# pierrepaleo/sift_pyocl

Measured on AMD Instinct MI355X. Metric: SiftPlan.keypoints throughput, 4096x4096 fp32 (Mpix/s; keypoints/s in keypoints_per_s), higher is better.
Workload: dtype f32

## Files before the change

include/siftmi.h:

```cpp
#ifndef SIFTMI_H
#define SIFTMI_H

#include <stdint.h>

#ifdef __cplusplus
extern "C" {
#endif

#define SIFTMI_OK 0
#define SIFTMI_EINVAL (-1)
#define SIFTMI_ENOMEM (-2)
#define SIFTMI_EDEVICE (-3)
#define SIFTMI_ECAPACITY (-4)

enum siftmi_dtype {
    SIFTMI_F32 = 0, SIFTMI_U8 = 1, SIFTMI_U16 = 2, SIFTMI_U32 = 3, SIFTMI_U64 = 4,
    SIFTMI_I32 = 5, SIFTMI_I64 = 6, SIFTMI_F64 = 7, SIFTMI_RGB8 = 8
};

typedef struct siftmi_keypoint {
    float x, y, scale, angle;
    uint8_t desc[128];
} siftmi_keypoint;

// ... 203 lines not shown
int siftmi_stage_dog(int32_t device_id, const float *blur_a, const float *blur_b, float *out, int64_t n);
int siftmi_stage_local_maxmin(int32_t device_id, const float *blurs, int32_t W, int32_t H, int32_t octsize,
                              const siftmi_params *params, float *out, int64_t capacity, int64_t *n_out);
int siftmi_stage_interp(int32_t device_id, const float *blurs, int32_t W, int32_t H, const float *cand, int64_t n,
                        const siftmi_params *params, float *out, int32_t *out_scale, int64_t *n_out);
#define SIFTMI_STAGE_GUARD 64
int siftmi_stage_detect_ex(int32_t device_id, const float *blurs, int32_t W, int32_t H, int32_t octsize,
                           const siftmi_params *params, int32_t form, int32_t rows, int32_t xcd_map, int32_t y_lo, int32_t y_hi,
                           int64_t cand_capacity, int64_t kp_capacity, float *cand, float *kp, int32_t *kp_aux,
                           int32_t *counters);
#define SIFTMI_STAGE_TOP_FILL 0x7fc5a5a5u
int siftmi_stage_detect_lazy(int32_t device_id, const float *blurs5, const float *top_taps, int32_t n_taps, int32_t W, int32_t H,
                             int32_t octsize, const siftmi_params *params, int32_t rows, int32_t xcd_map, int32_t y_lo, int32_t y_hi,
                             int64_t cand_capacity, int64_t kp_capacity, float *cand, float *kp, int32_t *kp_aux,
                             int32_t *counters, float *plane5);
int siftmi_stage_compact(int32_t device_id, const float *kps, int64_t n, int64_t start, int64_t end, float *out, int64_t *n_out);
int siftmi_stage_gradient(int32_t device_id, const float *img, float *grad, float *ori, int32_t W, int32_t H);
int siftmi_stage_orientation(int32_t device_id, const float *blurs, int32_t W, int32_t H, int32_t octsize,
                             const float *kps, const int32_t *kp_scale, int64_t n, const siftmi_params *params,
                             float *out, int32_t *out_scale, int64_t capacity, int64_t *n_out);
int siftmi_stage_descriptor(int32_t device_id, const float *blurs, int32_t W, int32_t H, int32_t octsize,
                            const float *kps, const int32_t *kp_scale, int64_t n, uint8_t *desc);
int siftmi_stage_orientation_ex(int32_t device_id, const float *blurs, int32_t W, int32_t H, int32_t octsize,
                                const float *kps, const int32_t *kp_scale, int64_t n, const siftmi_params *params,
                                float *out, int32_t *out_scale, int64_t capacity, int64_t *n_out,
                                int32_t form, int32_t blocks, int32_t *form_used);
int siftmi_stage_descriptor_ex(int32_t device_id, const float *blurs, int32_t W, int32_t H, int32_t octsize,
                               const float *kps, const int32_t *kp_scale, int64_t n, uint8_t *desc,
                               int32_t form, int32_t blocks, int32_t *form_used);
int siftmi_stage_gradient_maps(int32_t device_id, const float *planes, int32_t n_oct, const int32_t *W, const int32_t *H,
// ... 11 lines not shown
```

sift_pyocl_amd/_lib.py:

```python
import ctypes as C
import os
import subprocess

HERE = os.path.dirname(os.path.abspath(__file__))
LIB_PATH = os.path.join(HERE, "libsiftmi.so")

OK, EINVAL, ENOMEM, EDEVICE, ECAPACITY = 0, -1, -2, -3, -4
METRIC_L1, METRIC_L2SQ = 0, 1
INTERP_MODE, INTERP_CUBIC = 0, 1
INTERPS = {None: INTERP_MODE, "linear": INTERP_MODE, "cubic": INTERP_CUBIC}


def interp_code(interp, mode=1, rgb=False):
    if not (interp is None or isinstance(interp, str)) or interp not in INTERPS:
        raise ValueError("interp must be None, 'linear' or 'cubic', not %r" % (interp,))
    code = INTERPS[interp]
    if code == INTERP_CUBIC and int(mode) != 1:
        raise ValueError("interp='cubic' takes mode=1 only (other values are reserved), not %r" % (mode,))
    if code == INTERP_CUBIC and rgb:
        raise ValueError("interp='cubic' takes float32 frames; an RGB plan has no cubic sampler")
    return code


def interp_keyword(impl):
# ... 151 lines not shown
    "siftmi_stage_blur_ex": (C.c_int, [C.c_int32, C.c_void_p, C.c_int32, C.c_void_p, C.c_int32, C.c_int32, C.c_void_p, C.c_int32,
                                       C.c_int32, C.c_int32, C.c_int32, C.POINTER(C.c_int32)]),
    "siftmi_stage_blur_handoff": (C.c_int, [C.c_int32, C.c_void_p, C.c_void_p, C.c_void_p, C.c_int32, C.c_int32, C.c_void_p, C.c_int32,
                                            C.c_int32, C.c_int32, C.POINTER(C.c_int32)]),
    "siftmi_stage_dog": (C.c_int, [C.c_int32, C.c_void_p, C.c_void_p, C.c_void_p, C.c_int64]),
    "siftmi_stage_local_maxmin": (C.c_int, [C.c_int32, C.c_void_p, C.c_int32, C.c_int32, C.c_int32, C.POINTER(Params),
                                            C.c_void_p, C.c_int64, C.POINTER(C.c_int64)]),
    "siftmi_stage_interp": (C.c_int, [C.c_int32, C.c_void_p, C.c_int32, C.c_int32, C.c_void_p, C.c_int64,
                                      C.POINTER(Params), C.c_void_p, C.c_void_p, C.POINTER(C.c_int64)]),
    "siftmi_stage_detect_ex": (C.c_int, [C.c_int32, C.c_void_p, C.c_int32, C.c_int32, C.c_int32, C.POINTER(Params), C.c_int32,
                                         C.c_int32, C.c_int32, C.c_int32, C.c_int32, C.c_int64, C.c_int64, C.c_void_p, C.c_void_p,
                                         C.c_void_p, C.c_void_p]),
    "siftmi_stage_detect_lazy": (C.c_int, [C.c_int32, C.c_void_p, C.c_void_p, C.c_int32, C.c_int32, C.c_int32, C.c_int32, C.POINTER(Params),
                                           C.c_int32, C.c_int32, C.c_int32, C.c_int32, C.c_int64, C.c_int64, C.c_void_p, C.c_void_p,
                                           C.c_void_p, C.c_void_p, C.c_void_p]),
    "siftmi_stage_compact": (C.c_int, [C.c_int32, C.c_void_p, C.c_int64, C.c_int64, C.c_int64, C.c_void_p, C.POINTER(C.c_int64)]),
    "siftmi_stage_gradient": (C.c_int, [C.c_int32, C.c_void_p, C.c_void_p, C.c_void_p, C.c_int32, C.c_int32]),
    "siftmi_stage_orientation": (C.c_int, [C.c_int32, C.c_void_p, C.c_int32, C.c_int32, C.c_int32, C.c_void_p,
                                           C.c_void_p, C.c_int64, C.POINTER(Params), C.c_void_p, C.c_void_p,
                                           C.c_int64, C.POINTER(C.c_int64)]),
    "siftmi_stage_descriptor": (C.c_int, [C.c_int32, C.c_void_p, C.c_int32, C.c_int32, C.c_int32, C.c_void_p,
                                          C.c_void_p, C.c_int64, C.c_void_p]),
    "siftmi_stage_orientation_ex": (C.c_int, [C.c_int32, C.c_void_p, C.c_int32, C.c_int32, C.c_int32, C.c_void_p,
                                              C.c_void_p, C.c_int64, C.POINTER(Params), C.c_void_p, C.c_void_p,
                                              C.c_int64, C.POINTER(C.c_int64), C.c_int32, C.c_int32, C.POINTER(C.c_int32)]),
    "siftmi_stage_descriptor_ex": (C.c_int, [C.c_int32, C.c_void_p, C.c_int32, C.c_int32, C.c_int32, C.c_void_p,
                                             C.c_void_p, C.c_int64, C.c_void_p, C.c_int32, C.c_int32, C.POINTER(C.c_int32)]),
    "siftmi_stage_gradient_maps": (C.c_int, [C.c_int32, C.c_void_p, C.c_int32, C.c_void_p, C.c_void_p, C.c_int32,
                                             C.c_int32, C.c_int32, C.c_void_p, C.c_void_p]),
    "siftmi_plan_records_device": (C.c_int, [C.c_void_p, C.POINTER(C.c_void_p), C.POINTER(C.c_int64)]),
# ... 96 lines not shown
```

sift_pyocl_amd/csrc/k_extrema.hpp:

```cpp
#pragma once
#include <hip/hip_runtime.h>
#include <stdint.h>
#include "siftmath.hpp"
#include "k_xcd.hpp"
#include <type_traits>

namespace siftk {

struct BlurPlanes { const float *p[6]; };

#define SIFT_EXT_ROWS 64
inline int extrema_strip_rows(int W, int H, int border, int min_strips = 2000) {
    const int nx = (W - 2 * border + 61) / 62;
    int rows = SIFT_EXT_ROWS;
    while (rows > 4 && (int64_t)nx * ((H - 2 * border + rows - 1) / rows) < min_strips) rows >>= 1;
    return rows;
}

__device__ __forceinline__ float dog_at(const BlurPlanes &b, int s, size_t pos) { return b.p[s][pos] - b.p[s + 1][pos]; }

#ifndef SIFT_EXT_WAVES
#define SIFT_EXT_WAVES 5
#endif
#define SIFT_EXT_BUF 128
template <int BUF> struct ExtWaveLdsT { float4 buf[BUF + 192]; };
using ExtWaveLds = ExtWaveLdsT<SIFT_EXT_BUF>;

struct RefineArgs {
    float peak_thresh, init_sigma;
    float4 *kp;
    int *kp_aux, *n_kp;
    int kp_capacity, oct;
    int *c_scale;
};
__device__ __forceinline__ void refine_candidates(const BlurPlanes &b, int W, int H, const float4 *__restrict__ cand, int n,
                                                  float peak_thresh, float init_sigma, float4 *__restrict__ kp,
                                                  int *__restrict__ kp_aux, int *__restrict__ n_kp, int kp_capacity, int oct,
                                                  int first, int stride, int *__restrict__ c_scale);

template <int BUF>
__device__ __forceinline__ void ext_store_pending(const ExtWaveLdsT<BUF> &L, float4 *__restrict__ cand, int capacity, int slot, int count, int lane) {
    __builtin_amdgcn_wave_barrier();
    for (int e = lane; e < count; e += 64)
        if (slot + e < capacity) cand[slot + e] = L.buf[e];
    __builtin_amdgcn_wave_barrier();
}

template <int BUF>
__device__ __forceinline__ void ext_edge_filter(const BlurPlanes &b, int W, float edth, ExtWaveLdsT<BUF> &L, int from, int &pending, int lane) {
    int out = from;
    __builtin_amdgcn_wave_barrier();
    for (int base = from; base < pending; base += 64) {
        const int e = base + lane;
        bool keep = false;
        float4 c = make_float4(0.f, 0.f, 0.f, 0.f);
        if (e < pending) {
            c = L.buf[e];
            const float val = c.x;
            const int s = (int)c.w;
// ... 106 lines not shown
        for (int k = 0; k < 3; k++) {
            const unsigned long long m = __ballot(found[k]);
            if (m) {
                if (found[k]) L.buf[pending + __popcll(m & ((1ull << lane) - 1ull))] = make_float4(ctr[k], (float)yc, (float)x, (float)(k + 1));
                pending += __popcll(m);
            }
        }
        if (pending > BUF) {
            ext_edge_filter(b, W, edth, L, tested, pending, lane);
            tested = 0;
            if (REFINE) refine_parked();
            else {
                int slot = 0;
                if (lane == 0) slot = atomicAdd(counter, pending);
                ext_store_pending(L, cand, capacity, __shfl(slot, 0), pending, lane);
                pending = 0;
            }
        }
#pragma unroll
        for (int k = 0; k < 3; k++) ctr[k] = ctr_next[k];
    }
    ext_edge_filter(b, W, edth, L, tested, pending, lane);
    if (REFINE) refine_parked();
}

template <bool REFINE, bool LAZY = false>
__global__ __launch_bounds__(256) __attribute__((amdgpu_waves_per_eu(REFINE ? 4 : SIFT_EXT_WAVES, 8))) void extrema_kernel(BlurPlanes b, int W, int H, int border, int rows, double contrast,
                                                      float edth, float4 *__restrict__ cand,
                                                      int *__restrict__ counter, int capacity, RefineArgs ra,
                                                      int y_lo, int y_hi,
// ... 12 lines not shown
    extrema_strip<SIFT_EXT_BUF, REFINE, LAZY>(b, W, H, border, rows, active, active ? wid % nx : 0, active ? wid / nx : 0, contrast, edth, cand,
                                        counter, capacity, L, pending, &ra, y_lo, y_hi);
    if (REFINE) return;
    if (lane == 0) s_pending[threadIdx.x >> 6] = pending;
    __syncthreads();
    if (threadIdx.x == 0) {
        const int tot = s_pending[0] + s_pending[1] + s_pending[2] + s_pending[3];
        s_base = tot ? atomicAdd(counter, tot) : 0;
    }
    __syncthreads();
    {
        const int w = threadIdx.x >> 6;
        int slot = s_base;
        for (int q = 0; q < w; q++) slot += s_pending[q];
        ext_store_pending(L, cand, capacity, slot, pending, lane);
    }
}

__device__ __forceinline__ void refine_candidates(const BlurPlanes &b, int W, int H, const float4 *__restrict__ cand, int n,
                                                  float peak_thresh, float init_sigma, float4 *__restrict__ kp,
                                                  int *__restrict__ kp_aux, int *__restrict__ n_kp, int kp_capacity, int oct,
                                                  int first, int stride, int *__restrict__ c_scale) {
    int seen[3] = {0, 0, 0};
    for (int i = first; i < n; i += stride) {
        const float4 k = cand[i];
        int r = (int)k.y, c = (int)k.z;
        const int scale = (int)k.w;
        if (r == -1) continue;
        seen[0] += scale <= 1; seen[1] += scale == 2; seen[2] += scale >= 3;
        const float *Pa = b.p[0], *Pb = b.p[1], *Pc = b.p[2], *Pd = b.p[3];
// ... 101 lines not shown
```

sift_pyocl_amd/csrc/k_keypoint.hpp:

```cpp
#pragma once
#include <hip/hip_runtime.h>
#include <stdint.h>
#include "k_extrema.hpp"
#include "siftmath.hpp"

namespace siftk {

struct KpRecord { float x, y, scale, angle; uint8_t desc[128]; };
static_assert(sizeof(KpRecord) == 144, "record layout");

struct GradTaps { float xa, xb, ya, yb; bool bx, by; };

__device__ __forceinline__ GradTaps gradient_fetch(const float *__restrict__ I, int x, int y, int W, int H) {
    const size_t pos = (size_t)y * W + x;
    GradTaps t;
    t.bx = (x == 0) || (x == W - 1);
    t.by = (y == 0) || (y == H - 1);
    t.xa = I[x == W - 1 ? pos : pos + 1];
    t.xb = I[x == 0 ? pos : pos - 1];
    t.ya = I[y == 0 ? pos : pos - W];
    t.yb = I[y == H - 1 ? pos : pos + W];
    return t;
}

// ... 18 lines not shown
    return q;
}

#define SIFT_MAX_OCTAVES 24
#define SIFT_GROUPS 3
struct Counters {
    int n_rec;
    int tail_timeout;
    unsigned rec_word[SIFT_GROUPS];
    int g_kp[SIFT_GROUPS];
    int g_out[SIFT_GROUPS];
    int desc_next[SIFT_GROUPS];
    int n_cand[SIFT_MAX_OCTAVES + 1];
    int c_scale[SIFT_MAX_OCTAVES][3];
    int o_scale[SIFT_MAX_OCTAVES][3];
    uint32_t mm[2];
    int tail_ready[8];
};

struct OctaveTable {
    const float *base;
    long long off[SIFT_MAX_OCTAVES];
    int W[SIFT_MAX_OCTAVES], H[SIFT_MAX_OCTAVES];
    const float *gmap, *omap;
};
__device__ __forceinline__ size_t map_offset(const OctaveTable &tab, int oct, int scale) {
    return (size_t)(tab.off[oct] / 2) + (size_t)(scale - 1) * tab.W[oct] * tab.H[oct];
}

struct alignas(16) RecordSink {
// ... 621 lines not shown
```

sift_pyocl_amd/csrc/k_top_patch.hpp:

```cpp
#pragma once
#include <hip/hip_runtime.h>
#include <stdint.h>
#include "k_pyramid.hpp"

namespace siftk {

#define SIFT_TOP_R 6
#define SIFT_TOP_P (2 * SIFT_TOP_R + 1)
struct TopTaps { float t[64]; };

inline size_t top_patch_lds_bytes(int n_taps) {
    const size_t win = (size_t)(SIFT_TOP_P - 1 + n_taps);
    return (win * win + win * SIFT_TOP_P + 64 + SIFT_TOP_P * SIFT_TOP_P) * sizeof(float);
}

__global__ __launch_bounds__(64) void top_patch_kernel(const float *__restrict__ p4, float *__restrict__ p5, int W, int H, TopTaps taps, int n_taps,
                                                       float4 *__restrict__ cand, const int *__restrict__ n_cand, int cand_capacity) {
    extern __shared__ float top_lds[];
    const int lane = threadIdx.x;
    const int C = (n_taps & 1) ? n_taps / 2 : n_taps / 2 - 1;
    const int WIN = SIFT_TOP_P - 1 + n_taps;
    float *win = top_lds;
    float *hb = win + WIN * WIN;
    float *tr = hb + WIN * SIFT_TOP_P;
    float *pt = tr + 64;
    if (lane < n_taps) tr[lane] = taps.t[n_taps - 1 - lane];
    const int n = min(*n_cand, cand_capacity);
    for (int i = blockIdx.x; i < n; i += gridDim.x) {
        const float4 k = cand[i];
        const int r = __builtin_amdgcn_readfirstlane((int)k.y), c = __builtin_amdgcn_readfirstlane((int)k.z);
        if (__builtin_amdgcn_readfirstlane((int)k.w) != 3 || r == -1) continue;
        __syncthreads();
        const int y0 = r - SIFT_TOP_R, x0 = c - SIFT_TOP_R;
        for (int wc = lane; wc < WIN; wc += 64) {
            const float *col = p4 + reflect_index(x0 - C + wc, W);
#pragma unroll 8
            for (int wr = 0; wr < WIN; wr++) win[wr * WIN + wc] = col[(size_t)reflect_index(y0 - C + wr, H) * W];
        }
        __syncthreads();
        for (int base = 0; base < WIN * SIFT_TOP_P; base += 64 * 4) {
            const float *src[4];
            float a[4];
#pragma unroll
            for (int j = 0; j < 4; j++) {
                const int idx = min(base + 64 * j + lane, WIN * SIFT_TOP_P - 1);
                const int wr = idx / SIFT_TOP_P;
                src[j] = win + wr * WIN + (idx - wr * SIFT_TOP_P);
                a[j] = 0.0f;
            }
            for (int q = 0; q < n_taps; q++) {
                const float t = tr[q];
#pragma unroll
// ... 42 lines not shown
```

sift_pyocl_amd/csrc/siftmi.hip:

```cpp
#include <hip/hip_runtime.h>
#include <hip/hip_ext.h>

#include <cmath>
#include <cstdlib>
#include <cstring>
#include <algorithm>
#include <chrono>
#include <mutex>
#include <new>
#include <string>
#include <vector>

#include "host_common.hpp"
#include "k_extrema.hpp"
#include "k_keypoint.hpp"
#include "k_descriptor.hpp"
#include "k_align.hpp"
#include "k_align_batch.hpp"
#include "k_warp_cubic.hpp"
#include "k_stack.hpp"
#include "k_stack_clip.hpp"
#include "k_stack_accum.hpp"
#include "k_pyramid.hpp"
#include "k_tail.hpp"
// ... 88 lines not shown
size_t dtype_size(int dt) {
    switch (dt) {
        case SIFTMI_F32: return 4; case SIFTMI_U8: return 1; case SIFTMI_U16: return 2; case SIFTMI_U32: return 4;
        case SIFTMI_U64: return 8; case SIFTMI_I32: return 4; case SIFTMI_I64: return 8; case SIFTMI_F64: return 8;
        case SIFTMI_RGB8: return 3;
    }
    return 0;
}

}

struct GroupLists {
    float4 *kp = nullptr;  int *kp_aux = nullptr;  int64_t cap_kp = 0;
    float4 *okp = nullptr; int *oaux = nullptr;    int64_t cap_out = 0;
    float4 *cand = nullptr; int64_t cap_cand = 0;
};

struct siftmi_plan {
    void *chain = nullptr;
    int device = 0;
    hipStream_t stream = nullptr;
    int H = 0, W = 0, dtype = 0;
    siftmi_params par{};
    Options opt;
    int profile = 0;
    int n_oct = 0;
    std::vector<int> ow, oh;
    int64_t kpsize = 0;
    int64_t bytes = 0;
    float *planes = nullptr;
// ... 49 lines not shown
    KpRecord *host_out = nullptr;
    int host_cap = 0;
    bool desc_rows = true;
    Taps taps[6];
    bool have_init = false;
    std::vector<Event> events;
    size_t n_events = 0;
    hipEvent_t ev_first = nullptr, ev_last[3] = {nullptr, nullptr, nullptr};
    float last_min = 0, last_max = 0;
    int64_t last_count = 0;
    int last_overflow = 0;
    bool last_valid = false;
    int last_tail_first = 0;
    int last_n_cand[SIFT_MAX_OCTAVES] = {0};
    int last_c_scale[SIFT_MAX_OCTAVES][3] = {{0}};
    bool lazy_cur[SIFT_MAX_OCTAVES] = {false}, lazy_last[SIFT_MAX_OCTAVES] = {false}, lazy_ran[SIFT_MAX_OCTAVES] = {false};
    bool lazy_seen = false, lazy_block = false;
    std::vector<void *> allocs;

    template <class T> int alloc(T **p, size_t nbytes) {
        void *q = nullptr;
        hipError_t e = hipMalloc(&q, nbytes ? nbytes : 16);
        if (e != hipSuccess) return fail(SIFTMI_ENOMEM, "hipMalloc(%zu bytes): %s", nbytes, hipGetErrorString(e));
        allocs.push_back(q);
        bytes += (int64_t)nbytes;
        *p = (T *)q;
        return SIFTMI_OK;
    }
    template <class T> int regrow(T **p, size_t old_bytes, size_t new_bytes) {
        void *q = nullptr;
// ... 211 lines not shown
    if (!(W > 2 * border && H > 2 * border)) return g;
    g.rows = rows_opt > 0 ? rows_opt : (min_strips > 0 ? extrema_strip_rows(W, H, border, min_strips) : extrema_strip_rows(W, H, border));
    const int nx = (W - 2 * border + 61) / 62, ny = ((y_lo >= 0 ? y_hi - y_lo : H - 2 * border) + g.rows - 1) / g.rows;
    g.blocks = (nx * ny + 3) / 4;
    return g;
}

void launch_extrema(hipStream_t st, bool refine, const DetectGeom &geo, const BlurPlanes &bp, int W, int H, int border, double contrast, float edth,
                    float4 *cand, int *n_cand, int cand_cap, const RefineArgs &ra, int y_lo, int y_hi, int xcd_map, bool lazy = false) {
    auto go = [&](auto kernel) {
        hipLaunchKernelGGL(kernel, dim3((unsigned)geo.blocks), dim3(256), 0, st, bp, W, H, border, geo.rows, contrast, edth, cand, n_cand, cand_cap, ra, y_lo, y_hi, xcd_map);
    };
    if (refine) go(extrema_kernel<true>); else if (lazy) go(extrema_kernel<false, true>); else go(extrema_kernel<false>);
}

int launch_top_patch(hipStream_t st, int blocks, const float *p4, float *p5, int W, int H, const Taps &t, float4 *cand, const int *n_cand, int cand_cap) {
    if (t.n < 1 || t.n > 64) return fail(SIFTMI_EINVAL, "top_patch_kernel takes 1..64 taps, not %d", t.n);
    TopTaps ta;
    for (int i = 0; i < 64; i++) ta.t[i] = i < t.n ? t.t[i] : 0.0f;
    hipLaunchKernelGGL(top_patch_kernel, dim3((unsigned)blocks), dim3(64), top_patch_lds_bytes(t.n), st, p4, p5, W, H, ta, t.n, cand, n_cand, cand_cap);
    return SIFTMI_OK;
}

void launch_refine(hipStream_t st, int blocks, const BlurPlanes &bp, int W, int H, const float4 *cand, const int *n_cand, int cand_cap, const RefineArgs &ra) {
    hipLaunchKernelGGL(refine_kernel, dim3((unsigned)blocks), dim3(256), 0, st, bp, W, H, cand, n_cand, cand_cap, ra.peak_thresh, ra.init_sigma, ra.kp, ra.kp_aux,
                       ra.n_kp, ra.kp_capacity, ra.oct, ra.c_scale);
}

void launch_orientation(hipStream_t st, bool maps, int grid, int lds_pad, const OctaveTable &tab, float ori_sigma, const float4 *kp, const int *kp_aux,
                        Counters *cnt, int group, int kp_cap, float4 *okp, int *oaux, int out_cap, int team_below, int small_blocks) {
    auto go = [&](auto kernel) {
        hipLaunchKernelGGL(kernel, dim3((unsigned)grid), dim3(256), (size_t)lds_pad, st, tab, ori_sigma, kp, kp_aux, cnt, group, kp_cap, okp, oaux, out_cap, team_below, small_blocks);
    };
    if (maps) go(orientation_kernel<true>); else go(orientation_kernel<false>);
}

enum DescForm { DESC_ROWS = 0, DESC_ROWS_MAPS = 1, DESC_STREAM = 2 };
// ... 71 lines not shown
        return std::min<int64_t>(limit, std::max<int64_t>(need + need / 4 + 64, cap));
    };
    for (int g = 0; g < SIFT_GROUPS; g++) {
        if (g == 1 && !forks) continue;
        GroupLists &G = p->grp[g];
        int64_t need_cand = p->kpsize, need_kp = p->kpsize, need_out = p->kpsize;
        if (c) {
            need_cand = 0;
            for (int o = 0; o < p->n_oct && o < SIFT_MAX_OCTAVES; o++) if (cand_group_of(p, o) == g) need_cand = std::max<int64_t>(need_cand, c->n_cand[o]);
            need_kp = c->g_kp[g]; need_out = c->g_out[g];
        }
        const int64_t cc = want(G.cap_cand, need_cand, list_limit(p, 0, g)), ck = want(G.cap_kp, need_kp, list_limit(p, 1, g)),
                      co = want(G.cap_out, need_out, list_limit(p, 2, g));
        int rc = SIFTMI_OK;
        if (cc != G.cap_cand || ck != G.cap_kp || co != G.cap_out) quiesce();
        if (cc != G.cap_cand) { if ((rc = p->regrow(&G.cand, (size_t)G.cap_cand * 16, (size_t)cc * 16))) return rc; G.cap_cand = cc; if (grown) *grown = true; }
        if (ck != G.cap_kp) {
            if ((rc = p->regrow(&G.kp, (size_t)G.cap_kp * 16, (size_t)ck * 16)) || (rc = p->regrow(&G.kp_aux, (size_t)G.cap_kp * 4, (size_t)ck * 4))) return rc;
            G.cap_kp = ck; if (grown) *grown = true;
        }
        if (co != G.cap_out) {
            if ((rc = p->regrow(&G.okp, (size_t)G.cap_out * 16, (size_t)co * 16)) || (rc = p->regrow(&G.oaux, (size_t)G.cap_out * 4, (size_t)co * 4))) return rc;
            G.cap_out = co; if (grown) *grown = true;
        }
    }
    const int64_t cr = want(p->cap_rec, c ? (int64_t)c->n_rec : p->kpsize, list_limit(p, 3, 0));
    if (cr != p->cap_rec) {
        quiesce();
        int rc = p->regrow(&p->records, (size_t)p->cap_rec * sizeof(KpRecord), (size_t)cr * sizeof(KpRecord));
        if (rc) return rc;
        p->cap_rec = cr; if (grown) *grown = true;
// ... 38 lines not shown
    char lab[96];
    BlurPlanes bp;
    for (int s = 0; s < 6; s++) bp.p[s] = p->plane(oct, s);
    const int border = p->par.border_dist;
    GroupLists &GC = p->grp[cand_group_of(p, oct)];
    const int ccap = (int)GC.cap_cand, kcap = (int)G.cap_kp;
    int *n_cand = &p->cnt->n_cand[oct];
    const DetectGeom geo = detect_geometry(W, H, border, p->opt.ext_rows, p->opt.ext_strips, -1, -1);
    if (!geo.blocks) return;
    const RefineArgs ra = {p->par.peak_thresh, (float)p->par.init_sigma, G.kp, G.kp_aux, &p->cnt->g_kp[g], kcap, oct, &p->cnt->c_scale[oct][0]};
    const bool fused = detect_fused(p, oct);
    const bool lazy = oct < SIFT_MAX_OCTAVES && p->lazy_cur[oct];
    {
        snprintf(lab, sizeof lab, fused ? "local_maxmin+interp_keypoint %d" : "local_maxmin %d", oct);
        Scope sc(p, lab, false, 0, st);
        launch_extrema(st, fused, geo, bp, W, H, border, contrast_threshold(p->par), octave_edge_thresh(p->par, 1 << oct), GC.cand, n_cand, ccap, ra, -1, -1, p->opt.xcd_map, lazy);
    }
    if (fused) return;
    if (lazy) {
        snprintf(lab, sizeof lab, "top_patch %d", oct);
        Scope sc(p, lab, false, 0, st);
        (void)launch_top_patch(st, p->opt.top_blocks, p->plane(oct, 4), p->plane(oct, 5), W, H, p->taps[4], GC.cand, n_cand, ccap);
    }
    snprintf(lab, sizeof lab, "interp_keypoint+compact %d", oct);
    Scope sc(p, lab, false, 0, st);
    launch_refine(st, 512, bp, W, H, GC.cand, n_cand, ccap, ra);
}

int tail_first_octave(const siftmi_plan *p) {
    if (!p->opt.tail || p->profile > 1 || p->n_oct < 2) return p->n_oct;
    for (int s = 0; s < 5; s++) {
        const int n = p->taps[s].n;
        if (n != 11 && n != 15 && n != 17 && n != 21 && n != 27) return p->n_oct;
    }
    const int last = p->n_oct - 1;
    if (p->ow[(size_t)last] < 14 || p->oh[(size_t)last] < 14) return p->n_oct;
    int first = p->n_oct;
// ... 203 lines not shown
}

int siftmi_plan_destroy(siftmi_plan *p) {
    if (!p) return SIFTMI_OK;
    hipSetDevice(p->device);
    if (p->stream) hipStreamSynchronize(p->stream);
    if (p->stream2) { hipStreamSynchronize(p->stream2); hipStreamDestroy(p->stream2); }
    if (p->stream3) { hipStreamSynchronize(p->stream3); hipStreamDestroy(p->stream3); }
    if (p->ev_p3) hipEventDestroy(p->ev_p3);
    if (p->ev_det2) hipEventDestroy(p->ev_det2);
    if (p->ev_early) hipEventDestroy(p->ev_early);
    if (p->ev_maps0) hipEventDestroy(p->ev_maps0);
    for (hipEvent_t e : p->ev_pyr) hipEventDestroy(e);
    for (void *q : p->allocs) hipFree(q);
    for (GroupLists &G : p->grp)
        for (void *q : {(void *)G.kp, (void *)G.kp_aux, (void *)G.okp, (void *)G.oaux, (void *)G.cand}) if (q) hipFree(q);
    if (p->records) hipFree(p->records);
    if (p->hb) hipHostFree(p->hb);
    if (p->ev_join) hipEventDestroy(p->ev_join);
    if (p->warp_in) hipFree(p->warp_in);
    if (p->warp_out) hipFree(p->warp_out);
    if (p->ev_wa) hipEventDestroy(p->ev_wa);
    if (p->ev_wb) hipEventDestroy(p->ev_wb);
    for (Event &e : p->events) { hipEventDestroy(e.a); hipEventDestroy(e.b); }
    if (p->ev_first) hipEventDestroy(p->ev_first);
    for (hipEvent_t e : p->ev_last) if (e) hipEventDestroy(e);
    if (p->stream) hipStreamDestroy(p->stream);
    delete p;
    return SIFTMI_OK;
}

// ... 422 lines not shown
    p->records_cut = false;
    if (ovf) { int rc = cap_octaves(p, hc, &n); if (rc) return rc; }
    if (p->profile == 1) {
        float tot = 0, bms = 0; int32_t bl = 0; double px = 0;
        if (siftmi_plan_last_kernel_ms(p, &tot, nullptr, nullptr, nullptr) == SIFTMI_OK && siftmi_plan_blur_ms(p, 0, &bms, &bl, &px) == SIFTMI_OK) {
            p->acc_calls++; p->acc_total_ms += tot; p->acc_b0_ms += bms; p->acc_b0_launches += bl; p->acc_b0_pixels += px;
        }
    }
    p->last_count = n;
    p->last_overflow = ovf;
    p->last_tail_first = p->tail_first_cur;
    for (int o = 0; o < SIFT_MAX_OCTAVES; o++) {
        p->last_n_cand[o] = hc.n_cand[o] + (o == 0 ? hc.n_cand[SIFT_MAX_OCTAVES] : 0);
        for (int s = 0; s < 3; s++) p->last_c_scale[o][s] = hc.c_scale[o][s];
        if (p->lazy_cur[o]) p->last_n_cand[o] = hc.c_scale[o][0] + hc.c_scale[o][1] + hc.c_scale[o][2];
        p->lazy_last[o] = p->lazy_ran[o] = p->lazy_cur[o];
    }
    p->lazy_seen = true;
    p->lazy_block = false;
    p->last_valid = true;
    p->last_group0 = (int)std::min<int64_t>(hc.g_out[0], n);
    p->last_group1 = (int)n - p->last_group0;
    *n_out = n;
    if (overflow) *overflow = ovf;
    return SIFTMI_OK;
}

int plan_run(siftmi_plan *p, const void *image, int32_t image_dtype, int32_t image_is_device, bool sync_device, int64_t *n, int32_t *ovf) {
    int rc = SIFTMI_OK, tail_retries = 0;
    for (int attempt = 0; attempt < 12; attempt++) {
// ... 1207 lines not shown
        launch_extrema(0, form == 1, geo, bp, W, H, border, contrast_threshold(*par), octave_edge_thresh(*par, octsize), c.as<float4>(),
                       &dc->n_cand[0], (int)cand_capacity, ra, yl, yh, xcd_map ? 1 : 0);
        if (form == 0) launch_refine(0, 512, bp, W, H, c.as<float4>(), &dc->n_cand[0], (int)cand_capacity, ra);
    }
    if ((rc = stage_end())) return rc;
    Counters hc;
    HIPCHK(hipMemcpy(&hc, cnt.p, sizeof hc, hipMemcpyDeviceToHost));
    counters[0] = hc.n_cand[0]; counters[1] = hc.g_kp[0];
    for (int s = 0; s < 3; s++) counters[2 + s] = hc.c_scale[0][s];
    HIPCHK(hipMemcpy(cand, c.p, cslots * 16, hipMemcpyDeviceToHost));
    HIPCHK(hipMemcpy(kp, k.p, kslots * 16, hipMemcpyDeviceToHost));
    HIPCHK(hipMemcpy(kp_aux, ka.p, kslots * 4, hipMemcpyDeviceToHost));
    return SIFTMI_OK;
}

int siftmi_stage_detect_lazy(int32_t dev, const float *blurs5, const float *top_taps, int32_t n_taps, int32_t W, int32_t H, int32_t octsize,
                             const siftmi_params *par, int32_t rows, int32_t xcd_map, int32_t y_lo, int32_t y_hi,
                             int64_t cand_capacity, int64_t kp_capacity, float *cand, float *kp, int32_t *kp_aux, int32_t *counters, float *plane5) {
    int rc = stage_begin(dev); if (rc) return rc;
    if (!blurs5 || !top_taps || !par || !counters || !cand || !kp || !kp_aux || !plane5) return fail(SIFTMI_EINVAL, "null argument");
    if (W < 1 || H < 1) return fail(SIFTMI_EINVAL, "empty plane");
    if (n_taps < 1 || n_taps > 64) return fail(SIFTMI_EINVAL, "1..64 taps, not %d", n_taps);
    if (rows < 0 || rows > 4096) return fail(SIFTMI_EINVAL, "strip rows must be in 0..4096 (0: by the size rule)");
    if (cand_capacity < 0 || kp_capacity < 0 || cand_capacity > (1 << 30) || kp_capacity > (1 << 30)) return fail(SIFTMI_EINVAL, "capacity out of range");
    const int border = par->border_dist;
    if (border < 1) return fail(SIFTMI_EINVAL, "border_dist must be at least 1 (the 3 x 3 neighbourhood)");
    const bool band = y_lo >= 0;
    if (band && !(y_lo >= border && y_lo < y_hi && y_hi <= H - border))
        return fail(SIFTMI_EINVAL, "band [%d, %d) outside the detection rows [%d, %d)", y_lo, y_hi, border, H - border);
    int oct;
    if ((rc = stage_octave(octsize, oct))) return rc;
    const size_t N = (size_t)W * H;
    const size_t cslots = (size_t)cand_capacity + SIFTMI_STAGE_GUARD, kslots = (size_t)kp_capacity + SIFTMI_STAGE_GUARD;
    DevBuf b, c, k, ka, cnt;
    if ((rc = b.alloc(6 * N * 4)) || (rc = c.alloc(cslots * 16)) || (rc = k.alloc(kslots * 16)) ||
        (rc = ka.alloc(kslots * 4)) || (rc = cnt.alloc(sizeof(Counters)))) return rc;
    HIPCHK(hipMemcpy(b.p, blurs5, 5 * N * 4, hipMemcpyHostToDevice));
    HIPCHK(hipMemset(cnt.p, 0, sizeof(Counters)));
    {
        std::vector<uint32_t> fill(N, SIFTMI_STAGE_TOP_FILL);
        HIPCHK(hipMemcpy(b.as<float>() + 5 * N, fill.data(), N * 4, hipMemcpyHostToDevice));
        std::vector<float> holes(cslots * 4, -1.0f);
        HIPCHK(hipMemcpy(c.p, holes.data(), cslots * 16, hipMemcpyHostToDevice));
    }
    HIPCHK(hipMemset(k.p, 0xa5, kslots * 16));
    HIPCHK(hipMemset(ka.p, 0xa5, kslots * 4));
    BlurPlanes bp;
    for (int s = 0; s < 6; s++) bp.p[s] = b.as<float>() + (size_t)s * N;
    Counters *dc = cnt.as<Counters>();
    const int yl = band ? y_lo : -1, yh = band ? y_hi : -1;
    const DetectGeom geo = detect_geometry(W, H, border, rows, g_default_options.ext_strips, yl, yh);
    if (geo.blocks) {
        Taps tp;
        tp.n = n_taps;
        for (int i = 0; i < n_taps; i++) tp.t[i] = top_taps[i];
        const RefineArgs ra = {par->peak_thresh, (float)par->init_sigma, k.as<float4>(), ka.as<int>(), &dc->g_kp[0], (int)kp_capacity, oct, &dc->c_scale[0][0]};
        launch_extrema(0, false, geo, bp, W, H, border, contrast_threshold(*par), octave_edge_thresh(*par, octsize), c.as<float4>(),
                       &dc->n_cand[0], (int)cand_capacity, ra, yl, yh, xcd_map ? 1 : 0, true);
        if ((rc = launch_top_patch(0, g_default_options.top_blocks, bp.p[4], b.as<float>() + 5 * N, W, H, tp, c.as<float4>(), &dc->n_cand[0], (int)cand_capacity))) return rc;
        launch_refine(0, 512, bp, W, H, c.as<float4>(), &dc->n_cand[0], (int)cand_capacity, ra);
    }
    if ((rc = stage_end())) return rc;
    Counters hc;
    HIPCHK(hipMemcpy(&hc, cnt.p, sizeof hc, hipMemcpyDeviceToHost));
    counters[0] = hc.n_cand[0]; counters[1] = hc.g_kp[0];
    for (int s = 0; s < 3; s++) counters[2 + s] = hc.c_scale[0][s];
    HIPCHK(hipMemcpy(cand, c.p, cslots * 16, hipMemcpyDeviceToHost));
    HIPCHK(hipMemcpy(kp, k.p, kslots * 16, hipMemcpyDeviceToHost));
    HIPCHK(hipMemcpy(kp_aux, ka.p, kslots * 4, hipMemcpyDeviceToHost));
    HIPCHK(hipMemcpy(plane5, b.as<float>() + 5 * N, N * 4, hipMemcpyDeviceToHost));
    return SIFTMI_OK;
}

int siftmi_stage_compact(int32_t dev, const float *kps, int64_t n, int64_t start, int64_t end, float *out, int64_t *n_out) {
    int rc = stage_begin(dev); if (rc) return rc;
    if (!n_out || start < 0 || end < start || end > n) return fail(SIFTMI_EINVAL, "bad range");
    DevBuf a, o, cnt;
    if ((rc = a.upload(kps, (size_t)n * 16)) || (rc = o.alloc((size_t)n * 16)) || (rc = cnt.alloc(16))) return rc;
    HIPCHK(hipMemcpy(o.p, a.p, (size_t)start * 16, hipMemcpyDeviceToDevice));
    const int first = (int)start;
    HIPCHK(hipMemcpy(cnt.p, &first, 4, hipMemcpyHostToDevice));
    if (end > start)
        hipLaunchKernelGGL(compact_kernel, dim3(grid_for(end - start, 256, 1024)), dim3(256), 0, 0, (const float4 *)a.as<float4>(),
                           o.as<float4>(), cnt.as<int>(), (int)start, (int)end, (int)n);
    if ((rc = stage_end())) return rc;
    int count = 0;
// ... 165 lines not shown
```

Before: 23770.

## Emit compact top-scale candidate index list and size top_patch grid from it

```diff
diff --git a/include/siftmi.h b/include/siftmi.h
--- a/include/siftmi.h
+++ b/include/siftmi.h
@@ -241,6 +241,10 @@
                              int32_t octsize, const siftmi_params *params, int32_t rows, int32_t xcd_map, int32_t y_lo, int32_t y_hi,
                              int64_t cand_capacity, int64_t kp_capacity, float *cand, float *kp, int32_t *kp_aux,
                              int32_t *counters, float *plane5);
+int siftmi_stage_detect_lazy_list(int32_t device_id, const float *blurs5, const float *top_taps, int32_t n_taps, int32_t W, int32_t H,
+                                  int32_t octsize, const siftmi_params *params, int32_t rows, int32_t xcd_map, int32_t y_lo, int32_t y_hi,
+                                  int64_t cand_capacity, int64_t kp_capacity, float *cand, float *kp, int32_t *kp_aux,
+                                  int32_t *counters, float *plane5, int32_t *top_idx, int32_t *n_top, int32_t run_patch, int32_t top_blocks);
 int siftmi_stage_compact(int32_t device_id, const float *kps, int64_t n, int64_t start, int64_t end, float *out, int64_t *n_out);
 int siftmi_stage_gradient(int32_t device_id, const float *img, float *grad, float *ori, int32_t W, int32_t H);
 int siftmi_stage_orientation(int32_t device_id, const float *blurs, int32_t W, int32_t H, int32_t octsize,
diff --git a/sift_pyocl_amd/_lib.py b/sift_pyocl_amd/_lib.py
--- a/sift_pyocl_amd/_lib.py
+++ b/sift_pyocl_amd/_lib.py
@@ -189,6 +189,9 @@
     "siftmi_stage_detect_lazy": (C.c_int, [C.c_int32, C.c_void_p, C.c_void_p, C.c_int32, C.c_int32, C.c_int32, C.c_int32, C.POINTER(Params),
                                            C.c_int32, C.c_int32, C.c_int32, C.c_int32, C.c_int64, C.c_int64, C.c_void_p, C.c_void_p,
                                            C.c_void_p, C.c_void_p, C.c_void_p]),
+    "siftmi_stage_detect_lazy_list": (C.c_int, [C.c_int32, C.c_void_p, C.c_void_p, C.c_int32, C.c_int32, C.c_int32, C.c_int32, C.POINTER(Params),
+                                                C.c_int32, C.c_int32, C.c_int32, C.c_int32, C.c_int64, C.c_int64, C.c_void_p, C.c_void_p,
+                                                C.c_void_p, C.c_void_p, C.c_void_p, C.c_void_p, C.POINTER(C.c_int32), C.c_int32, C.c_int32]),
     "siftmi_stage_compact": (C.c_int, [C.c_int32, C.c_void_p, C.c_int64, C.c_int64, C.c_int64, C.c_void_p, C.POINTER(C.c_int64)]),
     "siftmi_stage_gradient": (C.c_int, [C.c_int32, C.c_void_p, C.c_void_p, C.c_void_p, C.c_int32, C.c_int32]),
     "siftmi_stage_orientation": (C.c_int, [C.c_int32, C.c_void_p, C.c_int32, C.c_int32, C.c_int32, C.c_void_p,
diff --git a/sift_pyocl_amd/csrc/k_extrema.hpp b/sift_pyocl_amd/csrc/k_extrema.hpp
--- a/sift_pyocl_amd/csrc/k_extrema.hpp
+++ b/sift_pyocl_amd/csrc/k_extrema.hpp
@@ -33,6 +33,13 @@
     int kp_capacity, oct;
     int *c_scale;
 };
+inline RefineArgs top_list_args(int *top_idx, int *n_top) {
+    RefineArgs a{};
+    a.kp_aux = top_idx; a.n_kp = n_top;
+    return a;
+}
+__device__ __forceinline__ int *top_idx_of(const RefineArgs &a) { return a.kp_aux; }
+__device__ __forceinline__ int *n_top_of(const RefineArgs &a) { return a.n_kp; }
 __device__ __forceinline__ void refine_candidates(const BlurPlanes &b, int W, int H, const float4 *__restrict__ cand, int n,
                                                   float peak_thresh, float init_sigma, float4 *__restrict__ kp,
                                                   int *__restrict__ kp_aux, int *__restrict__ n_kp, int kp_capacity, int oct,
@@ -43,6 +50,28 @@
     __builtin_amdgcn_wave_barrier();
     for (int e = lane; e < count; e += 64)
         if (slot + e < capacity) cand[slot + e] = L.buf[e];
+    __builtin_amdgcn_wave_barrier();
+}
+
+template <int BUF>
+__device__ __forceinline__ bool ext_is_top(const ExtWaveLdsT<BUF> &L, int capacity, int slot, int count, int e) {
+    return e < count && slot + e < capacity && L.buf[e].w == 3.0f;
+}
+template <int BUF>
+__device__ __forceinline__ int ext_count_top(const ExtWaveLdsT<BUF> &L, int capacity, int slot, int count, int lane) {
+    int n3 = 0;
+    __builtin_amdgcn_wave_barrier();
+    for (int base = 0; base < count; base += 64) n3 += __popcll(__ballot(ext_is_top(L, capacity, slot, count, base + lane)));
+    return n3;
+}
+template <int BUF>
+__device__ __forceinline__ void ext_store_top(const ExtWaveLdsT<BUF> &L, int *__restrict__ top_idx, int capacity, int slot, int count, int t0, int lane) {
+    for (int base = 0; base < count; base += 64) {
+        const bool top = ext_is_top(L, capacity, slot, count, base + lane);
+        const unsigned long long m = __ballot(top);
+        if (top) top_idx[t0 + __popcll(m & ((1ull << lane) - 1ull))] = slot + base + lane;
+        t0 += __popcll(m);
+    }
     __builtin_amdgcn_wave_barrier();
 }
 
@@ -179,6 +208,15 @@
                 int slot = 0;
                 if (lane == 0) slot = atomicAdd(counter, pending);
                 ext_store_pending(L, cand, capacity, __shfl(slot, 0), pending, lane);
+                if constexpr (LAZY) {
+                    slot = __shfl(slot, 0);
+                    const int n3 = ext_count_top(L, capacity, slot, pending, lane);
+                    if (n3) {
+                        int t0 = 0;
+                        if (lane == 0) t0 = atomicAdd(n_top_of(*ra), n3);
+                        ext_store_top(L, top_idx_of(*ra), capacity, slot, pending, __shfl(t0, 0), lane);
+                    }
+                }
                 pending = 0;
             }
         }
@@ -221,6 +259,20 @@
         int slot = s_base;
         for (int q = 0; q < w; q++) slot += s_pending[q];
         ext_store_pending(L, cand, capacity, slot, pending, lane);
+        if constexpr (LAZY) {
+            __shared__ int s_top[4], s_tbase;
+            const int n3 = ext_count_top(L, capacity, slot, pending, lane);
+            if (lane == 0) s_top[w] = n3;
+            __syncthreads();
+            if (threadIdx.x == 0) {
+                const int tot = s_top[0] + s_top[1] + s_top[2] + s_top[3];
+                s_tbase = tot ? atomicAdd(n_top_of(ra), tot) : 0;
+            }
+            __syncthreads();
+            int t0 = s_tbase;
+            for (int q = 0; q < w; q++) t0 += s_top[q];
+            ext_store_top(L, top_idx_of(ra), capacity, slot, pending, t0, lane);
+        }
     }
 }
 
diff --git a/sift_pyocl_amd/csrc/k_keypoint.hpp b/sift_pyocl_amd/csrc/k_keypoint.hpp
--- a/sift_pyocl_amd/csrc/k_keypoint.hpp
+++ b/sift_pyocl_amd/csrc/k_keypoint.hpp
@@ -56,6 +56,7 @@
     int n_cand[SIFT_MAX_OCTAVES + 1];
     int c_scale[SIFT_MAX_OCTAVES][3];
     int o_scale[SIFT_MAX_OCTAVES][3];
+    int n_top[SIFT_MAX_OCTAVES + 1];
     uint32_t mm[2];
     int tail_ready[8];
 };
diff --git a/sift_pyocl_amd/csrc/k_top_patch.hpp b/sift_pyocl_amd/csrc/k_top_patch.hpp
--- a/sift_pyocl_amd/csrc/k_top_patch.hpp
+++ b/sift_pyocl_amd/csrc/k_top_patch.hpp
@@ -14,8 +14,9 @@
     return (win * win + win * SIFT_TOP_P + 64 + SIFT_TOP_P * SIFT_TOP_P) * sizeof(float);
 }
 
+#define SIFT_TOP_LOADS 24
 __global__ __launch_bounds__(64) void top_patch_kernel(const float *__restrict__ p4, float *__restrict__ p5, int W, int H, TopTaps taps, int n_taps,
-                                                       float4 *__restrict__ cand, const int *__restrict__ n_cand, int cand_capacity) {
+                                                       const int *__restrict__ top_idx, const int *__restrict__ n_top, float4 *__restrict__ cand, int cand_capacity) {
     extern __shared__ float top_lds[];
     const int lane = threadIdx.x;
     const int C = (n_taps & 1) ? n_taps / 2 : n_taps / 2 - 1;
@@ -24,18 +25,31 @@
     float *hb = win + WIN * WIN;
     float *tr = hb + WIN * SIFT_TOP_P;
     float *pt = tr + 64;
+    const int n = min(*n_top, cand_capacity);
+    if ((int)blockIdx.x >= n) return;
     if (lane < n_taps) tr[lane] = taps.t[n_taps - 1 - lane];
-    const int n = min(*n_cand, cand_capacity);
-    for (int i = blockIdx.x; i < n; i += gridDim.x) {
+    const int row0 = lane / WIN, col0 = lane - row0 * WIN, srow = 64 / WIN, scol = 64 - srow * WIN;
+    for (int e = blockIdx.x; e < n; e += gridDim.x) {
+        const int i = top_idx[e];
         const float4 k = cand[i];
         const int r = __builtin_amdgcn_readfirstlane((int)k.y), c = __builtin_amdgcn_readfirstlane((int)k.z);
-        if (__builtin_amdgcn_readfirstlane((int)k.w) != 3 || r == -1) continue;
         __syncthreads();
         const int y0 = r - SIFT_TOP_R, x0 = c - SIFT_TOP_R;
-        for (int wc = lane; wc < WIN; wc += 64) {
-            const float *col = p4 + reflect_index(x0 - C + wc, W);
-#pragma unroll 8
-            for (int wr = 0; wr < WIN; wr++) win[wr * WIN + wc] = col[(size_t)reflect_index(y0 - C + wr, H) * W];
+        {
+            int wr = row0, wc = col0;
+            for (int base = lane; base < WIN * WIN; base += 64 * SIFT_TOP_LOADS) {
+                float v[SIFT_TOP_LOADS];
+                int at = base;
+#pragma unroll
+                for (int u = 0; u < SIFT_TOP_LOADS; u++) {
+                    v[u] = p4[(size_t)reflect_index(y0 - C + wr, H) * W + reflect_index(x0 - C + wc, W)];
+                    wr += srow; wc += scol;
+                    if (wc >= WIN) { wc -= WIN; wr++; }
+                }
+#pragma unroll
+                for (int u = 0; u < SIFT_TOP_LOADS; u++, at += 64)
+                    if (at < WIN * WIN) win[at] = v[u];
+            }
         }
         __syncthreads();
         for (int base = 0; base < WIN * SIFT_TOP_P; base += 64 * 4) {
diff --git a/sift_pyocl_amd/csrc/siftmi.hip b/sift_pyocl_amd/csrc/siftmi.hip
--- a/sift_pyocl_amd/csrc/siftmi.hip
+++ b/sift_pyocl_amd/csrc/siftmi.hip
@@ -126,6 +126,7 @@
     float4 *kp = nullptr;  int *kp_aux = nullptr;  int64_t cap_kp = 0;
     float4 *okp = nullptr; int *oaux = nullptr;    int64_t cap_out = 0;
     float4 *cand = nullptr; int64_t cap_cand = 0;
+    int *top_idx = nullptr;
 };
 
 struct siftmi_plan {
@@ -205,6 +206,7 @@
     int last_tail_first = 0;
     int last_n_cand[SIFT_MAX_OCTAVES] = {0};
     int last_c_scale[SIFT_MAX_OCTAVES][3] = {{0}};
+    int last_n_top[SIFT_MAX_OCTAVES] = {0};
     bool lazy_cur[SIFT_MAX_OCTAVES] = {false}, lazy_last[SIFT_MAX_OCTAVES] = {false}, lazy_ran[SIFT_MAX_OCTAVES] = {false};
     bool lazy_seen = false, lazy_block = false;
     std::vector<void *> allocs;
@@ -446,13 +448,14 @@
     if (refine) go(extrema_kernel<true>); else if (lazy) go(extrema_kernel<false, true>); else go(extrema_kernel<false>);
 }
 
-int launch_top_patch(hipStream_t st, int blocks, const float *p4, float *p5, int W, int H, const Taps &t, float4 *cand, const int *n_cand, int cand_cap) {
+int launch_top_patch(hipStream_t st, int blocks, const float *p4, float *p5, int W, int H, const Taps &t, const int *top_idx, const int *n_top, float4 *cand, int cand_cap) {
     if (t.n < 1 || t.n > 64) return fail(SIFTMI_EINVAL, "top_patch_kernel takes 1..64 taps, not %d", t.n);
     TopTaps ta;
     for (int i = 0; i < 64; i++) ta.t[i] = i < t.n ? t.t[i] : 0.0f;
-    hipLaunchKernelGGL(top_patch_kernel, dim3((unsigned)blocks), dim3(64), top_patch_lds_bytes(t.n), st, p4, p5, W, H, ta, t.n, cand, n_cand, cand_cap);
-    return SIFTMI_OK;
-}
+    hipLaunchKernelGGL(top_patch_kernel, dim3((unsigned)blocks), dim3(64), top_patch_lds_bytes(t.n), st, p4, p5, W, H, ta, t.n, top_idx, n_top, cand, cand_cap);
+    return SIFTMI_OK;
+}
+int top_patch_grid(int expected, int most) { return std::max(1, std::min(most, std::max(64, expected + expected / 4 + 32))); }
 
 void launch_refine(hipStream_t st, int blocks, const BlurPlanes &bp, int W, int H, const float4 *cand, const int *n_cand, int cand_cap, const RefineArgs &ra) {
     hipLaunchKernelGGL(refine_kernel, dim3((unsigned)blocks), dim3(256), 0, st, bp, W, H, cand, n_cand, cand_cap, ra.peak_thresh, ra.init_sigma, ra.kp, ra.kp_aux,
@@ -554,7 +557,10 @@
                       co = want(G.cap_out, need_out, list_limit(p, 2, g));
         int rc = SIFTMI_OK;
         if (cc != G.cap_cand || ck != G.cap_kp || co != G.cap_out) quiesce();
-        if (cc != G.cap_cand) { if ((rc = p->regrow(&G.cand, (size_t)G.cap_cand * 16, (size_t)cc * 16))) return rc; G.cap_cand = cc; if (grown) *grown = true; }
+        if (cc != G.cap_cand) {
+            if ((rc = p->regrow(&G.cand, (size_t)G.cap_cand * 16, (size_t)cc * 16)) || (rc = p->regrow(&G.top_idx, (size_t)G.cap_cand * 4, (size_t)cc * 4))) return rc;
+            G.cap_cand = cc; if (grown) *grown = true;
+        }
         if (ck != G.cap_kp) {
             if ((rc = p->regrow(&G.kp, (size_t)G.cap_kp * 16, (size_t)ck * 16)) || (rc = p->regrow(&G.kp_aux, (size_t)G.cap_kp * 4, (size_t)ck * 4))) return rc;
             G.cap_kp = ck; if (grown) *grown = true;
@@ -623,13 +629,15 @@
     {
         snprintf(lab, sizeof lab, fused ? "local_maxmin+interp_keypoint %d" : "local_maxmin %d", oct);
         Scope sc(p, lab, false, 0, st);
-        launch_extrema(st, fused, geo, bp, W, H, border, contrast_threshold(p->par), octave_edge_thresh(p->par, 1 << oct), GC.cand, n_cand, ccap, ra, -1, -1, p->opt.xcd_map, lazy);
+        launch_extrema(st, fused, geo, bp, W, H, border, contrast_threshold(p->par), octave_edge_thresh(p->par, 1 << oct), GC.cand, n_cand, ccap,
+                       lazy ? top_list_args(GC.top_idx, &p->cnt->n_top[oct]) : ra, -1, -1, p->opt.xcd_map, lazy);
     }
     if (fused) return;
     if (lazy) {
         snprintf(lab, sizeof lab, "top_patch %d", oct);
         Scope sc(p, lab, false, 0, st);
-        (void)launch_top_patch(st, p->opt.top_blocks, p->plane(oct, 4), p->plane(oct, 5), W, H, p->taps[4], GC.cand, n_cand, ccap);
+        (void)launch_top_patch(st, top_patch_grid(p->last_n_top[oct], p->opt.top_blocks), p->plane(oct, 4), p->plane(oct, 5), W, H, p->taps[4], GC.top_idx,
+                               &p->cnt->n_top[oct], GC.cand, ccap);
     }
     snprintf(lab, sizeof lab, "interp_keypoint+compact %d", oct);
     Scope sc(p, lab, false, 0, st);
@@ -863,7 +871,7 @@
     for (hipEvent_t e : p->ev_pyr) hipEventDestroy(e);
     for (void *q : p->allocs) hipFree(q);
     for (GroupLists &G : p->grp)
-        for (void *q : {(void *)G.kp, (void *)G.kp_aux, (void *)G.okp, (void *)G.oaux, (void *)G.cand}) if (q) hipFree(q);
+        for (void *q : {(void *)G.kp, (void *)G.kp_aux, (void *)G.okp, (void *)G.oaux, (void *)G.cand, (void *)G.top_idx}) if (q) hipFree(q);
     if (p->records) hipFree(p->records);
     if (p->hb) hipHostFree(p->hb);
     if (p->ev_join) hipEventDestroy(p->ev_join);
@@ -1316,6 +1324,7 @@
         p->last_n_cand[o] = hc.n_cand[o] + (o == 0 ? hc.n_cand[SIFT_MAX_OCTAVES] : 0);
         for (int s = 0; s < 3; s++) p->last_c_scale[o][s] = hc.c_scale[o][s];
         if (p->lazy_cur[o]) p->last_n_cand[o] = hc.c_scale[o][0] + hc.c_scale[o][1] + hc.c_scale[o][2];
+        p->last_n_top[o] = p->lazy_cur[o] ? hc.n_top[o] : (int)std::min<int64_t>(2 * (int64_t)hc.c_scale[o][2], 1 << 30);
         p->lazy_last[o] = p->lazy_ran[o] = p->lazy_cur[o];
     }
     p->lazy_seen = true;
@@ -2553,11 +2562,13 @@
     return SIFTMI_OK;
 }
 
-int siftmi_stage_detect_lazy(int32_t dev, const float *blurs5, const float *top_taps, int32_t n_taps, int32_t W, int32_t H, int32_t octsize,
-                             const siftmi_params *par, int32_t rows, int32_t xcd_map, int32_t y_lo, int32_t y_hi,
-                             int64_t cand_capacity, int64_t kp_capacity, float *cand, float *kp, int32_t *kp_aux, int32_t *counters, float *plane5) {
+int siftmi_stage_detect_lazy_list(int32_t dev, const float *blurs5, const float *top_taps, int32_t n_taps, int32_t W, int32_t H, int32_t octsize,
+                                  const siftmi_params *par, int32_t rows, int32_t xcd_map, int32_t y_lo, int32_t y_hi,
+                                  int64_t cand_capacity, int64_t kp_capacity, float *cand, float *kp, int32_t *kp_aux, int32_t *counters, float *plane5,
+                                  int32_t *top_idx, int32_t *n_top, int32_t run_patch, int32_t top_blocks) {
     int rc = stage_begin(dev); if (rc) return rc;
-    if (!blurs5 || !top_taps || !par || !counters || !cand || !kp || !kp_aux || !plane5) return fail(SIFTMI_EINVAL, "null argument");
+    if (!blurs5 || !top_taps || !par || !counters || !cand || !kp || !kp_aux || !plane5 || !top_idx || !n_top) return fail(SIFTMI_EINVAL, "null argument");
+    if (top_blocks < 0 || top_blocks > 65535) return fail(SIFTMI_EINVAL, "top_patch_kernel takes at most 65535 workgroups");
     if (W < 1 || H < 1) return fail(SIFTMI_EINVAL, "empty plane");
     if (n_taps < 1 || n_taps > 64) return fail(SIFTMI_EINVAL, "1..64 taps, not %d", n_taps);
     if (rows < 0 || rows > 4096) return fail(SIFTMI_EINVAL, "strip rows must be in 0..4096 (0: by the size rule)");
@@ -2571,8 +2582,8 @@
     if ((rc = stage_octave(octsize, oct))) return rc;
     const size_t N = (size_t)W * H;
     const size_t cslots = (size_t)cand_capacity + SIFTMI_STAGE_GUARD, kslots = (size_t)kp_capacity + SIFTMI_STAGE_GUARD;
-    DevBuf b, c, k, ka, cnt;
-    if ((rc = b.alloc(6 * N * 4)) || (rc = c.alloc(cslots * 16)) || (rc = k.alloc(kslots * 16)) ||
+    DevBuf b, c, ti, k, ka, cnt;
+    if ((rc = b.alloc(6 * N * 4)) || (rc = c.alloc(cslots * 16)) || (rc = ti.alloc(cslots * 4)) || (rc = k.alloc(kslots * 16)) ||
         (rc = ka.alloc(kslots * 4)) || (rc = cnt.alloc(sizeof(Counters)))) return rc;
     HIPCHK(hipMemcpy(b.p, blurs5, 5 * N * 4, hipMemcpyHostToDevice));
     HIPCHK(hipMemset(cnt.p, 0, sizeof(Counters)));
@@ -2582,6 +2593,7 @@
         std::vector<float> holes(cslots * 4, -1.0f);
         HIPCHK(hipMemcpy(c.p, holes.data(), cslots * 16, hipMemcpyHostToDevice));
     }
+    HIPCHK(hipMemset(ti.p, 0xa5, cslots * 4));
     HIPCHK(hipMemset(k.p, 0xa5, kslots * 16));
     HIPCHK(hipMemset(ka.p, 0xa5, kslots * 4));
     BlurPlanes bp;
@@ -2595,9 +2607,12 @@
         for (int i = 0; i < n_taps; i++) tp.t[i] = top_taps[i];
         const RefineArgs ra = {par->peak_thresh, (float)par->init_sigma, k.as<float4>(), ka.as<int>(), &dc->g_kp[0], (int)kp_capacity, oct, &dc->c_scale[0][0]};
         launch_extrema(0, false, geo, bp, W, H, border, contrast_threshold(*par), octave_edge_thresh(*par, octsize), c.as<float4>(),
-                       &dc->n_cand[0], (int)cand_capacity, ra, yl, yh, xcd_map ? 1 : 0, true);
-        if ((rc = launch_top_patch(0, g_default_options.top_blocks, bp.p[4], b.as<float>() + 5 * N, W, H, tp, c.as<float4>(), &dc->n_cand[0], (int)cand_capacity))) return rc;
-        launch_refine(0, 512, bp, W, H, c.as<float4>(), &dc->n_cand[0], (int)cand_capacity, ra);
+                       &dc->n_cand[0], (int)cand_capacity, top_list_args(ti.as<int>(), &dc->n_top[0]), yl, yh, xcd_map ? 1 : 0, true);
+        if (run_patch) {
+            if ((rc = launch_top_patch(0, top_blocks ? top_blocks : g_default_options.top_blocks, bp.p[4], b.as<float>() + 5 * N, W, H, tp, ti.as<int>(), &dc->n_top[0],
+                                       c.as<float4>(), (int)cand_capacity))) return rc;
+            launch_refine(0, 512, bp, W, H, c.as<float4>(), &dc->n_cand[0], (int)cand_capacity, ra);
+        }
     }
     if ((rc = stage_end())) return rc;
     Counters hc;
@@ -2608,7 +2623,19 @@
     HIPCHK(hipMemcpy(kp, k.p, kslots * 16, hipMemcpyDeviceToHost));
     HIPCHK(hipMemcpy(kp_aux, ka.p, kslots * 4, hipMemcpyDeviceToHost));
     HIPCHK(hipMemcpy(plane5, b.as<float>() + 5 * N, N * 4, hipMemcpyDeviceToHost));
-    return SIFTMI_OK;
+    HIPCHK(hipMemcpy(top_idx, ti.p, cslots * 4, hipMemcpyDeviceToHost));
+    *n_top = hc.n_top[0];
+    return SIFTMI_OK;
+}
+
+int siftmi_stage_detect_lazy(int32_t dev, const float *blurs5, const float *top_taps, int32_t n_taps, int32_t W, int32_t H, int32_t octsize,
+                             const siftmi_params *par, int32_t rows, int32_t xcd_map, int32_t y_lo, int32_t y_hi,
+                             int64_t cand_capacity, int64_t kp_capacity, float *cand, float *kp, int32_t *kp_aux, int32_t *counters, float *plane5) {
+    if (cand_capacity < 0 || cand_capacity > (1 << 30)) return fail(SIFTMI_EINVAL, "capacity out of range");
+    std::vector<int32_t> top_idx((size_t)cand_capacity + SIFTMI_STAGE_GUARD);
+    int32_t n_top = 0;
+    return siftmi_stage_detect_lazy_list(dev, blurs5, top_taps, n_taps, W, H, octsize, par, rows, xcd_map, y_lo, y_hi, cand_capacity, kp_capacity, cand, kp, kp_aux,
+                                         counters, plane5, top_idx.data(), &n_top, 1, 0);
 }
 
 int siftmi_stage_compact(int32_t dev, const float *kps, int64_t n, int64_t start, int64_t end, float *out, int64_t *n_out) {
```

Result: no change. 23710 (-0.2%).
